# ypw0102/GDR

Measured on AMD Instinct MI355X. Metric: queries/sec on NQ-320k (768-d), higher is better.
Workload: dtype f32; 1 GPU; C2/ragged/prefilter: t5-base encoder 512 q/GPU + Q.D^T top-100, 320000x768 corpus; batch_per_gpu=512, global_batch=512, seq_len=40, corpus_rows=320000, dim=768, k=100, encoder_rows=ragged

## Files before the change

gdr_amd/csrc/encoder.hip:

```cpp
#include <stdlib.h>

#include "layers.h"

namespace gdr {

constexpr size_t ENC_SPLITK_BYTES = (size_t)112 << 20;
static_assert(STREAMK_BYTES <= ENC_SPLITK_BYTES, "stream-K scratch must fit the split-K region");

static int enc_streamk(char* splitk_region, StreamK* sk, hipStream_t stream) {
  sk->part = reinterpret_cast<float*>(splitk_region);
  sk->flag = reinterpret_cast<int32_t*>(splitk_region + STREAMK_PART_BYTES);
  sk->epoch = 0;
  if (hipMemsetAsync(sk->flag, 0, 512 * sizeof(int32_t), stream) != hipSuccess) {
    set_error("t5_encoder: memset of the stream-K flags failed");
    return GDR_EHIP;
  }
  return GDR_OK;
}

struct EncWs {
  size_t off_h, off_nx, off_qkv, off_ctx, off_ff, off_splitk, off_bf, total;
};

static EncWs enc_ws(const GdrT5Dims& dm, int64_t M, bool bf16 = false) {
// ... 97 lines not shown
        const __bf16* q16 = reinterpret_cast<const __bf16*>(qkv);
        at.q = reinterpret_cast<const float*>(q16), at.k = reinterpret_cast<const float*>(q16 + inner);
        at.v = reinterpret_cast<const float*>(q16 + 2 * inner), at.qkv_bf16 = 1;
      }
      at.out_bf16 = abf;
      if ((rc = launch_attention(at, stream))) return rc;
      if ((rc = lin16(abf, ly.wo, h, d, d, inner, 0, h, 0))) return rc;
      if ((rc = launch_rmsnorm_bf16(h, ly.ln_ff, abf, M, d, dm.eps, stream))) return rc;
      if ((rc = lin16(abf, ly.wi, ff, dm.d_ff, dm.d_ff, d, 1, nullptr, 1))) return rc;
      if ((rc = lin16(ff, ly.wo_ff, h, d, d, dm.d_ff, 0, h, 0))) return rc;
      continue;
    }
    if ((rc = launch_rmsnorm(h, ly.ln_attn, nx, M, d, dm.eps, nullptr, 1, stream))) return rc;
    if ((rc = linear(nx, d, ly.wqkv, qkv, 3 * inner, 3 * inner, d, GDR_EPI_NONE, nullptr))) return rc;
    if ((rc = launch_attention(at, stream))) return rc;
    if ((rc = linear(ctx, inner, ly.wo, h, d, d, inner, GDR_EPI_RESIDUAL, h))) return rc;
    if ((rc = launch_rmsnorm(h, ly.ln_ff, nx, M, d, dm.eps, nullptr, 1, stream))) return rc;
    if ((rc = linear(nx, d, ly.wi, ff, dm.d_ff, dm.d_ff, d, GDR_EPI_RELU, nullptr))) return rc;
    if ((rc = linear(ff, dm.d_ff, ly.wo_ff, h, d, d, dm.d_ff, GDR_EPI_RESIDUAL, h))) return rc;
  }
  return launch_rmsnorm(h, w->final_ln, out_hidden, M, d, dm.eps, out_pooled, L, stream);
}
}

extern "C" int gdr_t5_encoder_forward(const GdrT5EncoderWeights* w, const int64_t* ids, const int64_t* mask, int B,
                                      int L, float* out_hidden, float* out_pooled, void* workspace,
                                      size_t workspace_bytes, void* stream_) {
  return gdr::t5_encoder_impl(w, ids, mask, B, L, out_hidden, out_pooled, workspace, workspace_bytes, false,
                              static_cast<hipStream_t>(stream_));
}

namespace gdr {
struct RagWs {
  size_t seq_len, seq_off, row_src, rows_total, ctx_cls, h_cls, nx_cls, ff_cls, total;
};
static RagWs rag_ws(const GdrT5Dims& dm, int B, int L, size_t base) {
  RagWs r{};
  const size_t inner = (size_t)dm.num_heads * dm.d_kv;
  size_t o = base;
  r.seq_len = o, o += align_up((size_t)B * 4, 256);
  r.seq_off = o, o += align_up((size_t)(B + 1) * 4, 256);
  r.row_src = o, o += align_up((size_t)B * L * 4, 256);
  r.rows_total = o, o += 256;
  r.ctx_cls = o, o += align_up((size_t)B * inner * 4, 256);
  r.h_cls = o, o += align_up((size_t)B * dm.d_model * 4, 256);
  r.nx_cls = o, o += align_up((size_t)B * dm.d_model * 4, 256);
  r.ff_cls = o, o += align_up((size_t)B * dm.d_ff * 4, 256);
  r.total = o;
  return r;
}
static bool ragged_packs(const GdrT5Dims& dm, int B, int L) {
  const int64_t tiles = (((int64_t)B * L + 127) / 128) * ((dm.d_model + 127) / 128);
  return dm.d_kv == 64 && tiles >= 192 && dm.d_model % 32 == 0 && dm.d_ff % 32 == 0 && (dm.num_heads * dm.d_kv) % 32 == 0;
}
static bool ragged_packs_small(const GdrT5Dims& dm, int B, int L) {
  return dm.d_kv == 64 && (int64_t)B * L >= 256 && dm.d_model % 32 == 0 && dm.d_ff % 32 == 0 && (dm.num_heads * dm.d_kv) % 32 == 0;
}
}

extern "C" size_t gdr_t5_encoder_ragged_workspace_bytes(const GdrT5Dims* dims, int B, int L) {
  if (!dims || B <= 0 || L <= 0) return 0;
  return gdr::rag_ws(*dims, B, L, gdr::enc_ws(*dims, (int64_t)B * L, true).total).total;
}

namespace gdr {
static int ragged_impl(const GdrT5EncoderWeights* w, const int64_t* ids, const int64_t* mask, int B, int L, float* out_hidden,
                       float* out_pooled, int64_t live_rows_hint, void* workspace, size_t workspace_bytes, bool bf16,
                       hipStream_t stream) {
  if (B == 0) return GDR_OK;
  GDR_CHECK_ARG(w && ids && mask && workspace && (out_hidden || out_pooled), "t5_encoder_ragged: null pointer");
  const GdrT5Dims& dm = w->dims;
  GDR_CHECK_ARG(B > 0 && L > 0 && L <= 128, "t5_encoder_ragged: B=%d L=%d (L must be in [1,128])", B, L);
  GDR_CHECK_ARG(dm.d_model % 4 == 0 && dm.d_kv % 4 == 0 && dm.d_ff % 4 == 0, "t5_encoder_ragged: dims must be multiples of 4");
  GDR_CHECK_ARG(w->embed && w->rel_bias && w->final_ln && w->layers, "t5_encoder_ragged: null weight pointer");
  const int64_t M = (int64_t)B * L;
  const EncWs ws = enc_ws(dm, M, true);
  const RagWs rw = rag_ws(dm, B, L, ws.total);
  if (workspace_bytes < rw.total) {
    set_error("t5_encoder_ragged: workspace %zu < required %zu", workspace_bytes, rw.total);
    return GDR_ENOSPC;
// ... 65 lines not shown
          return rc;
        if ((rc = launch_gather_rows(h, seq_off, B, d, h_cls, stream))) return rc;
        if ((rc = lin16(ctx_cls16, ly.wo, h_cls, d, B, nullptr, d, inner, 0, h_cls, 0))) return rc;
        if ((rc = launch_rmsnorm_bf16(h_cls, ly.ln_ff, nx_cls16, B, d, dm.eps, stream))) return rc;
        if ((rc = lin16(nx_cls16, ly.wi, static_cast<float*>(ff_cls16), dm.d_ff, B, nullptr, dm.d_ff, d, 1, nullptr, 1))) return rc;
        if ((rc = lin16(ff_cls16, ly.wo_ff, h_cls, d, B, nullptr, d, dm.d_ff, 0, h_cls, 0))) return rc;
        return launch_rmsnorm(h_cls, w->final_ln, out_pooled, B, d, dm.eps, nullptr, 1, stream);
      }
      if ((rc = lin16(abf, ly.wo, h, d, M, rows_dev, d, inner, 0, h, 0))) return rc;
      if ((rc = launch_rmsnorm_bf16_dev(h, ly.ln_ff, abf, rows_dev, M, d, dm.eps, stream))) return rc;
      if ((rc = lin16(abf, ly.wi, ff, dm.d_ff, M, rows_dev, dm.d_ff, d, 1, nullptr, 1))) return rc;
      if ((rc = lin16(ff, ly.wo_ff, h, d, M, rows_dev, d, dm.d_ff, 0, h, 0))) return rc;
    }
    if ((rc = launch_rmsnorm_dev(h, w->final_ln, nx, rows_dev, M, d, dm.eps, stream))) return rc;
    if (out_pooled && (rc = launch_gather_rows(nx, seq_off, B, d, out_pooled, stream))) return rc;
    if (out_hidden) {
      if (hipMemsetAsync(out_hidden, 0, (size_t)M * d * sizeof(float), stream) != hipSuccess) {
        set_error("t5_encoder_ragged: memset failed");
        return GDR_EHIP;
      }
      if ((rc = launch_scatter_rows(nx, row_src, rows_dev, M, d, out_hidden, stream))) return rc;
    }
    return GDR_OK;
  }
  float* h = reinterpret_cast<float*>(base + ws.off_h);
  float* nx = reinterpret_cast<float*>(base + ws.off_nx);
  float* qkv = reinterpret_cast<float*>(base + ws.off_qkv);
  float* ctx = reinterpret_cast<float*>(base + ws.off_ctx);
  float* ff = reinterpret_cast<float*>(base + ws.off_ff);
  float* ctx_cls = reinterpret_cast<float*>(base + rw.ctx_cls);
  float* h_cls = reinterpret_cast<float*>(base + rw.h_cls);
  float* nx_cls = reinterpret_cast<float*>(base + rw.nx_cls);
  float* ff_cls = reinterpret_cast<float*>(base + rw.ff_cls);
  StreamK sk{};
  if ((rc = enc_streamk(base + ws.off_splitk, &sk, stream))) return rc;
  float* skw = reinterpret_cast<float*>(base + ws.off_splitk);
  auto linear = [&](const float* A, int64_t lda, const float* W, float* C, int64_t ldc, int N, int K, int epi,
                    const float* residual) -> int {
    if (small)
      return launch_linear_f32_ws(A, lda, W, K, C, ldc, M, N, K, epi, nullptr, residual, ldc, skw, ENC_SPLITK_BYTES, stream, &sk,
                                  rows_dev, live_rows_hint);
    return launch_linear_f32_dev(A, lda, W, K, C, ldc, M, rows_dev, N, K, epi, nullptr, residual, ldc, live_rows_hint, stream,
                                 &sk);
  };
  if ((rc = launch_embed_packed(w->embed, ids, row_src, rows_dev, M, d, dm.vocab_size, h, stream))) return rc;

  AttnArgs at{};
  at.q = qkv, at.k = qkv + inner, at.v = qkv + 2 * inner, at.out = ctx;
  at.ldq = at.ldk = at.ldv = 3 * inner, at.ldo = inner;
  at.q_bstride = at.k_bstride = at.o_bstride = L;
  at.B = B, at.H = H, at.dk = dk, at.Lq = L, at.Lk = L;
  at.q_pos0 = 0, at.scale = 1.0f;
  at.rel_bias = w->rel_bias, at.bidirectional = 1, at.num_buckets = dm.rel_buckets;
  at.lut = make_bucket_lut(dm.rel_buckets / 2, dm.rel_max_distance);
  at.key_mask = mask, at.mask_bstride = L, at.causal = 0, at.causal_neg_inf = 0;
  at.kv_rows = nullptr, at.kv_group = 1;
  at.seq_off = seq_off, at.seq_len = seq_len;

  const bool pooled_only = out_hidden == nullptr && big;
  for (int i = 0; i < dm.num_layers; ++i) {
    const GdrT5EncLayer& ly = w->layers[i];
    GDR_CHECK_ARG(ly.ln_attn && ly.wqkv && ly.wo && ly.ln_ff && ly.wi && ly.wo_ff, "t5_encoder_ragged: layer %d null weight", i);
    if ((rc = launch_rmsnorm_dev(h, ly.ln_attn, nx, rows_dev, M, d, dm.eps, stream))) return rc;
    if ((rc = linear(nx, d, ly.wqkv, qkv, 3 * inner, 3 * inner, d, GDR_EPI_NONE, nullptr))) return rc;
    if ((rc = launch_attention(at, stream))) return rc;
    if (pooled_only && i == dm.num_layers - 1) {
      if ((rc = launch_gather_rows(ctx, seq_off, B, inner, ctx_cls, stream))) return rc;
      if ((rc = launch_gather_rows(h, seq_off, B, d, h_cls, stream))) return rc;
      if ((rc = launch_linear_f32(ctx_cls, inner, ly.wo, inner, h_cls, d, B, d, inner, GDR_EPI_RESIDUAL, nullptr, h_cls, d, stream)))
        return rc;
      if ((rc = launch_rmsnorm(h_cls, ly.ln_ff, nx_cls, B, d, dm.eps, nullptr, 1, stream))) return rc;
      if ((rc = launch_linear_f32(nx_cls, d, ly.wi, d, ff_cls, dm.d_ff, B, dm.d_ff, d, GDR_EPI_RELU, nullptr, nullptr, 0, stream)))
        return rc;
      if ((rc = launch_linear_f32(ff_cls, dm.d_ff, ly.wo_ff, dm.d_ff, h_cls, d, B, d, dm.d_ff, GDR_EPI_RESIDUAL, nullptr, h_cls, d,
                                  stream)))
        return rc;
      return launch_rmsnorm(h_cls, w->final_ln, out_pooled, B, d, dm.eps, nullptr, 1, stream);
    }
    if ((rc = linear(ctx, inner, ly.wo, h, d, d, inner, GDR_EPI_RESIDUAL, h))) return rc;
    if ((rc = launch_rmsnorm_dev(h, ly.ln_ff, nx, rows_dev, M, d, dm.eps, stream))) return rc;
    if ((rc = linear(nx, d, ly.wi, ff, dm.d_ff, dm.d_ff, d, GDR_EPI_RELU, nullptr))) return rc;
    if ((rc = linear(ff, dm.d_ff, ly.wo_ff, h, d, d, dm.d_ff, GDR_EPI_RESIDUAL, h))) return rc;
  }
  if ((rc = launch_rmsnorm_dev(h, w->final_ln, nx, rows_dev, M, d, dm.eps, stream))) return rc;
  if (out_pooled && (rc = launch_gather_rows(nx, seq_off, B, d, out_pooled, stream))) return rc;
  if (out_hidden) {
    if (hipMemsetAsync(out_hidden, 0, (size_t)M * d * sizeof(float), stream) != hipSuccess) {
      set_error("t5_encoder_ragged: memset failed");
      return GDR_EHIP;
    }
    if ((rc = launch_scatter_rows(nx, row_src, rows_dev, M, d, out_hidden, stream))) return rc;
  }
  return GDR_OK;
}
}

namespace gdr {
static size_t split_ws_a_bytes(const GdrT5Dims& dm, int64_t M) {
  const int inner = dm.num_heads * dm.d_kv;
  int ld = split_row_elems(dm.d_model);
  if (split_row_elems(inner) > ld) ld = split_row_elems(inner);
  return align_up((size_t)M * ld * 2, 256);
}
static size_t split_ws_bytes(const GdrT5Dims& dm, int64_t M) {
  return split_ws_a_bytes(dm, M) + align_up((size_t)M * split_row_elems(dm.d_ff) * 2, 256);
}

static int ragged_split_impl(const GdrT5EncoderWeights* w, const int64_t* ids, const int64_t* mask, int B, int L, float* out_hidden,
                             float* out_pooled, int64_t live_rows_hint, int terms, void* workspace, size_t workspace_bytes,
                             hipStream_t stream) {
  if (B == 0) return GDR_OK;
// ... 161 lines not shown
```

gdr_amd/csrc/layers.h:

```cpp
#pragma once
#include "common.h"

namespace gdr {

struct BucketLut {
  uint8_t v[128];
};
BucketLut make_bucket_lut(int nb, int max_distance);

struct AttnArgs {
  const float* q;
  const float* k;
  const float* v;
  float* out;
  void* out_bf16;
  int64_t ldq, ldk, ldv, ldo;
  int64_t q_bstride, k_bstride, o_bstride;
  int B, H, dk, Lq, Lk;
  int q_pos0;
  float scale;
  const float* rel_bias;
  int bidirectional, num_buckets;
  BucketLut lut;
  const int64_t* key_mask;
  int64_t mask_bstride;
  int causal;
  int causal_neg_inf;
  const int32_t* kv_rows;
  int kv_group;
  int q_same_pos;
  const int32_t* seq_off;
  const int32_t* seq_len;
  int qkv_bf16;
  const int64_t* b_count_dev;
  const float* q_part;
  int q_S, q_tiles_n;
  const int32_t* live;
};
int launch_attention(const AttnArgs& a, hipStream_t stream);
int launch_attention_long(const AttnArgs& a, hipStream_t stream);

int launch_embed(const float* table, const int64_t* ids, int64_t rows, int d, int vocab, float* out,
                 hipStream_t stream);
int launch_pack_plan(const int64_t* mask, int B, int L, int32_t* seq_len, int32_t* seq_off, int32_t* row_src,
                     int64_t* rows_total, hipStream_t stream);
int launch_embed_packed(const float* table, const int64_t* ids, const int32_t* row_src, const int64_t* rows_dev,
                        int64_t max_rows, int d, int vocab, float* out, hipStream_t stream);
int launch_gather_rows(const float* src, const int32_t* idx, int n, int d, float* dst, hipStream_t stream);
int launch_scatter_rows(const float* src, const int32_t* row_src, const int64_t* rows_dev, int64_t max_rows, int d,
                        float* dst, hipStream_t stream);
int launch_rmsnorm(const float* x, const float* w, float* y, int64_t rows, int d, float eps, float* pooled,
                   int pool_every, hipStream_t stream, void* y16 = nullptr);
int launch_zero_dead_rows(float* x, const int32_t* seq_len, int B, int L, int d, hipStream_t stream);
int launch_rmsnorm_dev(const float* x, const float* w, float* y, const int64_t* rows_dev, int64_t max_rows, int d, float eps,
                       hipStream_t stream, void* y16 = nullptr);
int launch_rmsnorm_planes(const float* x, const float* w, float* y, void* planes, int64_t ld, const int64_t* rows_dev, int64_t max_rows,
                          int d, float eps, hipStream_t stream, int f16x2 = 0);
int launch_rmsnorm_bf16(const float* x, const float* w, void* y_bf16, int64_t rows, int d, float eps, hipStream_t stream);
int launch_rmsnorm_bf16_dev(const float* x, const float* w, void* y_bf16, const int64_t* rows_dev, int64_t max_rows, int d,
                            float eps, hipStream_t stream);
int launch_layernorm(const float* x, const float* w, const float* b, float* y, int64_t rows, int d, float eps,
                     const float* addv, hipStream_t stream, void* y16 = nullptr, int f16x2_ld = 0);
int launch_layernorm_dev(const float* x, const float* w, const float* b, float* y, const int64_t* rows_dev, int64_t max_rows,
                         int d, float eps, const float* addv, hipStream_t stream, void* y16 = nullptr, int f16x2_ld = 0);
int launch_layernorm2(const float* x, const float* w1, const float* b1, const float* w2, const float* b2, const float* addv, float* y,
                      const int64_t* rows_dev, int64_t max_rows, int d, float eps, hipStream_t stream, void* y16 = nullptr);
// ... 3 lines not shown
```

gdr_amd/csrc/layers.hip:

```cpp
#include <math.h>

#include <stdlib.h>

#include "layers.h"

namespace gdr {

BucketLut make_bucket_lut(int nb, int max_distance) {
  BucketLut l;
  const int max_exact = nb / 2;
  for (int n = 0; n < 128; ++n) {
    int b;
    if (n < max_exact) {
      b = n;
    } else {
      const float v = logf((float)n / (float)max_exact) / (float)log((double)max_distance / max_exact) *
                      (float)(nb - max_exact);
      b = max_exact + (int)v;
      if (b > nb - 1) b = nb - 1;
    }
    l.v[n] = (uint8_t)b;
  }
  return l;
}
// ... 611 lines not shown
        }
      }
      sum = wave_sum(sum);
      sc[0] = sum;
    }
    __builtin_amdgcn_wave_barrier();
    if (active) {
      const float inv = 1.0f / sc[0];
      float* orow = a.out + ((int64_t)b * a.o_bstride + i) * a.ldo + h * dk;
      for (int d = lane; d < dk; d += 64) {
        float o = 0.f;
        int j = 0;
        for (; j + 4 <= Lk; j += 4) {
          const float4 pp = *reinterpret_cast<const float4*>(ps + j);
          o = fmaf(pp.x * inv, Vs[(j + 0) * dks + d], o);
          o = fmaf(pp.y * inv, Vs[(j + 1) * dks + d], o);
          o = fmaf(pp.z * inv, Vs[(j + 2) * dks + d], o);
          o = fmaf(pp.w * inv, Vs[(j + 3) * dks + d], o);
        }
        for (; j < Lk; ++j) o = fmaf(ps[j] * inv, Vs[j * dks + d], o);
        if (a.out_bf16)
          static_cast<__bf16*>(a.out_bf16)[((int64_t)b * a.o_bstride + i) * a.ldo + h * dk + d] = (__bf16)o;
        else
          orow[d] = o;
      }
    }
    __builtin_amdgcn_wave_barrier();
  }
}


typedef float f32x4_t __attribute__((ext_vector_type(4)));

template <int NT>
__global__ __launch_bounds__(64 * NT) void attention_mfma16_kernel(const AttnArgs a) {
  extern __shared__ __attribute__((aligned(16))) float smem[];
  constexpr int DK = 64, DS = DK + 4, LP = 16 * NT, NTHR = 64 * NT;
  const int Lr = a.Lk;
  float* Ks = smem;
  float* Vs = Ks + Lr * DS;
  float* RelB = Vs + Lr * DS;
  float* Mk = RelB + 2 * LP;
  const int b = blockIdx.x / a.H, h = blockIdx.x % a.H;
  const int L = a.seq_len ? a.seq_len[b] : a.Lk, tid = threadIdx.x;
  const int64_t qrow0 = a.seq_off ? a.seq_off[b] : (int64_t)b * a.q_bstride;
  const int64_t krow0 = a.seq_off ? a.seq_off[b] : (int64_t)b * a.k_bstride;
  const int64_t orow0 = a.seq_off ? a.seq_off[b] : (int64_t)b * a.o_bstride;
  float4 qv[DK / 16];
  {
    const int wq = tid >> 6, lq = tid & 63;
    const int64_t qr = qrow0 + min(16 * wq + (lq & 15), L - 1);
    if (16 * wq < L) {
      if (a.qkv_bf16) {
        const __bf16* q16 = reinterpret_cast<const __bf16*>(a.q) + qr * a.ldq + h * DK + 4 * (lq >> 4);
#pragma unroll
        for (int jj = 0; jj < DK / 16; ++jj) {
          const uint2 u = *reinterpret_cast<const uint2*>(q16 + 16 * jj);
          qv[jj] = make_float4(__uint_as_float(u.x << 16) * a.scale, __uint_as_float(u.x & 0xffff0000u) * a.scale,
                               __uint_as_float(u.y << 16) * a.scale, __uint_as_float(u.y & 0xffff0000u) * a.scale);
        }
      } else {
        const float* q32 = a.q + qr * a.ldq + h * DK + 4 * (lq >> 4);
#pragma unroll
        for (int jj = 0; jj < DK / 16; ++jj) qv[jj] = *reinterpret_cast<const float4*>(q32 + 16 * jj);
      }
    }
  }
  int rb_bucket = -1;
  int rb_lutoff[2];
  unsigned char rb_lut[2] = {0, 0};
  int rb_base[2] = {0, 0};
  constexpr int RBI = (2 * LP + NTHR - 1) / NTHR;
  static_assert(RBI == 1, "one bias cell per thread");
  if (a.rel_bias && tid < 2 * LP) {
    int n = tid - (LP - 1), bucket = 0;
    if (a.bidirectional) {
      if (n < 0) {
        bucket = a.num_buckets >> 1;
        n = -n;
      }
    } else if (n < 0) {
      n = 0;
    }
    rb_base[0] = bucket;
    rb_lutoff[0] = n < 127 ? n : 127;
// ... 34 lines not shown
    }
    __builtin_amdgcn_sched_barrier(0);
    asm volatile("" ::: "memory");
    float rb_val = 0.f;
    if (rb_bucket >= 0) rb_val = a.rel_bias[(rb_base[0] + rb_lut[0]) * a.H + h];
    __builtin_amdgcn_sched_barrier(0);
    asm volatile("" ::: "memory");
#pragma unroll
    for (int it = 0; it < KI; ++it) {
      asm volatile("" : "+v"(kst[it].x), "+v"(kst[it].y), "+v"(kst[it].z), "+v"(kst[it].w));
      asm volatile("" : "+v"(vst[it].x), "+v"(vst[it].y), "+v"(vst[it].z), "+v"(vst[it].w));
    }
    asm volatile("" : "+v"(mk_raw));
#pragma unroll
    for (int it = 0; it < KI; ++it) {
      const int e = tid + it * NTHR;
      if (e < L * (DK / 4)) {
        const int r = e >> 4, c = e & 15;
        *reinterpret_cast<float4*>(Ks + r * DS + 4 * c) = kst[it];
        *reinterpret_cast<float4*>(Vs + r * DS + 4 * c) = vst[it];
      }
    }
    if (tid < 2 * LP) RelB[tid] = rb_val;
  }
  if (a.qkv_bf16 && tid < 2 * LP) RelB[tid] = rb_bucket >= 0 ? a.rel_bias[(rb_base[0] + rb_lut[0]) * a.H + h] : 0.f;
  if (tid < LP) Mk[tid] = tid < L ? ((mk_mine && mk_raw == 0) ? (a.causal_neg_inf ? -INFINITY : -1e9f) : 0.f) : -INFINITY;
  __syncthreads();
  if (!a.qkv_bf16) {
#pragma unroll
    for (int jj = 0; jj < DK / 16; ++jj) qv[jj].x *= a.scale, qv[jj].y *= a.scale, qv[jj].z *= a.scale, qv[jj].w *= a.scale;
  }

  const int w = tid >> 6, lane = tid & 63, c16 = lane & 15, q4 = lane >> 4;
  if (16 * w >= L) return;
  const int nt_live = (L + 15) >> 4;
  f32x4_t st[NT];
#pragma unroll
  for (int t = 0; t < NT; ++t) st[t] = (f32x4_t){0.f, 0.f, 0.f, 0.f};
#pragma unroll
  for (int jj = 0; jj < DK / 16; ++jj) {
#pragma unroll
    for (int t = 0; t < NT; ++t) {
      if (t >= nt_live) continue;
      const float4 kv = *reinterpret_cast<const float4*>(Ks + min(16 * t + c16, L - 1) * DS + 4 * q4 + 16 * jj);
      st[t] = __builtin_amdgcn_mfma_f32_16x16x4f32(kv.x, qv[jj].x, st[t], 0, 0, 0);
      st[t] = __builtin_amdgcn_mfma_f32_16x16x4f32(kv.y, qv[jj].y, st[t], 0, 0, 0);
      st[t] = __builtin_amdgcn_mfma_f32_16x16x4f32(kv.z, qv[jj].z, st[t], 0, 0, 0);
      st[t] = __builtin_amdgcn_mfma_f32_16x16x4f32(kv.w, qv[jj].w, st[t], 0, 0, 0);
    }
  }
  const int i = 16 * w + c16;
  const float masked = a.causal_neg_inf ? -INFINITY : -1e9f;
  float mx = -INFINITY;
#pragma unroll
  for (int t = 0; t < NT; ++t) {
    if (t >= nt_live) continue;
#pragma unroll
    for (int r = 0; r < 4; ++r) {
      const int j = 16 * t + 4 * q4 + r;
      float add = RelB[i - j + (LP - 1)] + Mk[j];
      if (a.causal && j > i && Mk[j] == 0.f) add += masked;
      const float s = st[t][r] + add;
      st[t][r] = s;
      mx = fmaxf(mx, s);
    }
  }
  mx = fmaxf(mx, __shfl_xor(mx, 16));
  mx = fmaxf(mx, __shfl_xor(mx, 32));
  float sum = 0.f;
#pragma unroll
  for (int t = 0; t < NT; ++t) {
    if (t >= nt_live) continue;
#pragma unroll
    for (int r = 0; r < 4; ++r) {
      const float p = __expf(st[t][r] - mx);
      st[t][r] = p;
      sum += p;
    }
  }
  sum += __shfl_xor(sum, 16);
  sum += __shfl_xor(sum, 32);
  const float inv = 1.0f / sum;
#pragma unroll
  for (int dt = 0; dt < DK / 16; ++dt) {
    f32x4_t o = (f32x4_t){0.f, 0.f, 0.f, 0.f};
#pragma unroll
    for (int t = 0; t < NT; ++t) {
      if (t >= nt_live) continue;
#pragma unroll
      for (int r = 0; r < 4; ++r) {
        const int j = 16 * t + 4 * q4 + r;
        const float vv = Vs[min(j, L - 1) * DS + 16 * dt + c16];
        o = __builtin_amdgcn_mfma_f32_16x16x4f32(vv, st[t][r], o, 0, 0, 0);
      }
    }
    if (i < L) {
      const int64_t off = (orow0 + i) * a.ldo + h * DK + 16 * dt + 4 * q4;
      const float4 ov = make_float4(o[0] * inv, o[1] * inv, o[2] * inv, o[3] * inv);
      if (a.out_bf16)
        *reinterpret_cast<uint2*>(static_cast<__bf16*>(a.out_bf16) + off) = pack_bf16x4(ov.x, ov.y, ov.z, ov.w);
      else
        *reinterpret_cast<float4*>(a.out + off) = ov;
    }
  }
}

typedef __bf16 bf16x8_t __attribute__((ext_vector_type(8)));

__device__ __forceinline__ uint32_t bf16_trunc_bits(float x) { return __float_as_uint(x) & 0xffff0000u; }

template <int NT>
__global__ __launch_bounds__(64 * NT) void attention_mfma_bf16_kernel(const AttnArgs a) {
  extern __shared__ __attribute__((aligned(16))) unsigned char smem_b[];
  constexpr int DK = 64, KS = 144, VS = 272, LP = 16 * NT, NTHR = 64 * NT, NB = (NT + 1) / 2, VKEYS = 32 * NB;
  const int Lr = a.Lk;
  unsigned char* Ks = smem_b;
  unsigned char* Vt = Ks + (size_t)((Lr * KS + 15) & ~15);
  float* RelB = reinterpret_cast<float*>(Vt + DK * VS);
  float* Mk = RelB + 2 * LP;
  const int b = blockIdx.x / a.H, h = blockIdx.x % a.H;
  const int L = a.seq_len ? a.seq_len[b] : a.Lk, tid = threadIdx.x;
  const int64_t qrow0 = a.seq_off ? a.seq_off[b] : (int64_t)b * a.q_bstride;
  const int64_t krow0 = a.seq_off ? a.seq_off[b] : (int64_t)b * a.k_bstride;
  const int64_t orow0 = a.seq_off ? a.seq_off[b] : (int64_t)b * a.o_bstride;
  const __bf16* q16 = reinterpret_cast<const __bf16*>(a.q);
  const __bf16* k16 = reinterpret_cast<const __bf16*>(a.k);
  const __bf16* v16 = reinterpret_cast<const __bf16*>(a.v);
  uint4 qv[2];
  {
    const int wq = tid >> 6, lq = tid & 63;
// ... 120 lines not shown
#pragma unroll
    for (int u = 0; u < NB; ++u) {
      if (2 * u >= nt_live) continue;
      const uint2 v0 = *reinterpret_cast<const uint2*>(vr + 64 * u);
      const uint2 v1 = *reinterpret_cast<const uint2*>(vr + 64 * u + 32);
      const bf16x8_t va = __builtin_bit_cast(bf16x8_t, make_uint4(v0.x, v0.y, v1.x, v1.y));
      o = __builtin_amdgcn_mfma_f32_16x16x32_bf16(va, __builtin_bit_cast(bf16x8_t, ph[u]), o, 0, 0, 0);
      o = __builtin_amdgcn_mfma_f32_16x16x32_bf16(va, __builtin_bit_cast(bf16x8_t, pm[u]), o, 0, 0, 0);
      o = __builtin_amdgcn_mfma_f32_16x16x32_bf16(va, __builtin_bit_cast(bf16x8_t, pl[u]), o, 0, 0, 0);
    }
    if (i < L) {
      const int64_t off = (orow0 + i) * a.ldo + h * DK + 16 * dt + 4 * q4;
      const float4 ov = make_float4(o[0] * inv, o[1] * inv, o[2] * inv, o[3] * inv);
      if (a.out_bf16)
        *reinterpret_cast<uint2*>(static_cast<__bf16*>(a.out_bf16) + off) = pack_bf16x4(ov.x, ov.y, ov.z, ov.w);
      else
        *reinterpret_cast<float4*>(a.out + off) = ov;
    }
  }
}

template <int NT>
static int launch_attention_mfma_bf16(const AttnArgs& a, hipStream_t stream) {
  const size_t lds = (size_t)((a.Lk * 144 + 15) & ~15) + 64 * 272 + sizeof(float) * 3 * 16 * NT;
  if (int rc__ = ensure_dyn_lds(reinterpret_cast<const void*>(attention_mfma_bf16_kernel<NT>), 160 * 1024, "attention")) return rc__;
  hipLaunchKernelGGL(attention_mfma_bf16_kernel<NT>, dim3((unsigned)(a.B * a.H)), dim3(64 * NT), lds, stream, a);
  GDR_CHECK_LAUNCH("attention_mfma_bf16_kernel");
  return GDR_OK;
}

template <int NT>
static int launch_attention_mfma16(const AttnArgs& a, hipStream_t stream) {
  const size_t lds = sizeof(float) * ((size_t)2 * a.Lk * 68 + 3 * 16 * NT);
  if (int rc__ = ensure_dyn_lds(reinterpret_cast<const void*>(attention_mfma16_kernel<NT>), 160 * 1024, "attention")) return rc__;
  hipLaunchKernelGGL(attention_mfma16_kernel<NT>, dim3((unsigned)(a.B * a.H)), dim3(64 * NT), lds, stream, a);
  GDR_CHECK_LAUNCH("attention_mfma16_kernel");
  return GDR_OK;
}


template <int NT>
__global__ __launch_bounds__(512) void attention_cross_mfma16_kernel(const AttnArgs a) {
  extern __shared__ __attribute__((aligned(16))) float smem[];
  if (a.live && *a.live == 0) return;
  constexpr int DK = 64, DS = DK + 4, LP = 16 * NT;
  const int Lk = a.Lk, Lq = a.Lq;
  float* Ks = smem;
  float* Vs = Ks + Lk * DS;
  float* Add = Vs + Lk * DS;
  const int b = blockIdx.x / a.H, h = blockIdx.x % a.H;
  const int tid = threadIdx.x, nthr = blockDim.x;
  const int w = tid >> 6, lane = tid & 63, c16 = lane & 15, q4 = lane >> 4;
  const int64_t krow0 = (int64_t)(b / a.kv_group) * a.k_bstride;
  float4 qv[DK / 16];
  const bool has_rows = 16 * w < Lq;
  if (has_rows) {
    const int64_t qr = (int64_t)b * a.q_bstride + min(16 * w + c16, Lq - 1);
    const float* q32 = a.q + qr * a.ldq + h * DK + 4 * q4;
#pragma unroll
    for (int jj = 0; jj < DK / 16; ++jj) {
      float4 t = *reinterpret_cast<const float4*>(q32 + 16 * jj);
      t.x *= a.scale, t.y *= a.scale, t.z *= a.scale, t.w *= a.scale;
      qv[jj] = t;
    }
  }
  for (int j = tid; j < LP; j += nthr) {
// ... 415 lines not shown
          hipLaunchKernelGGL(attention_decode_heads4_kernel<4>, g4, dim3(256), 0, stream, a);
        else if (a.Lk <= 8)
          hipLaunchKernelGGL(attention_decode_heads4_kernel<8>, g4, dim3(256), 0, stream, a);
        else if (a.Lk <= 12)
          hipLaunchKernelGGL(attention_decode_heads4_kernel<12>, g4, dim3(256), 0, stream, a);
        else
          hipLaunchKernelGGL(attention_decode_heads4_kernel<16>, g4, dim3(256), 0, stream, a);
        GDR_CHECK_LAUNCH("attention_decode_heads4_kernel");
        return GDR_OK;
      }
#endif
      const dim3 grids((unsigned)((a.B * a.H + 3) / 4));
      if (a.dk <= 64)
        hipLaunchKernelGGL(attention_decode_short_kernel<16>, grids, dim3(256), 0, stream, a);
      else
        hipLaunchKernelGGL(attention_decode_short_kernel<32>, grids, dim3(256), 0, stream, a);
      GDR_CHECK_LAUNCH("attention_decode_short_kernel");
      return GDR_OK;
    }
    const dim3 grid((unsigned)((a.B * a.H + 3) / 4));
    if (a.dk <= 64)
      hipLaunchKernelGGL(attention_decode_rows_kernel<16>, grid, dim3(256), 0, stream, a);
    else
      hipLaunchKernelGGL(attention_decode_rows_kernel<32>, grid, dim3(256), 0, stream, a);
    GDR_CHECK_LAUNCH("attention_decode_rows_kernel");
    return GDR_OK;
  }
  const bool packed = a.seq_off != nullptr || a.qkv_bf16;
  GDR_CHECK_ARG(!a.seq_off || a.seq_len, "attention: seq_off without seq_len");
  GDR_CHECK_ARG(!packed || (a.Lq == a.Lk && a.q_pos0 == 0 && !a.kv_rows && a.kv_group == 1 && !a.q_same_pos &&
                            a.dk == 64 && a.ldo % 4 == 0),
                "attention: the packed (ragged) form and bf16 q/k/v serve full self-attention with d_kv = 64 only");
  GDR_CHECK_ARG(!a.qkv_bf16 || (a.ldq % 8 == 0 && a.ldk % 8 == 0 && a.ldv % 8 == 0), "attention: bf16 q/k/v need row strides %% 8 == 0");
  if (a.Lq == a.Lk && a.q_pos0 == 0 && !a.kv_rows && a.kv_group == 1 && !a.q_same_pos && a.dk == 64 && a.ldo % 4 == 0) {
    if (a.Lk > 128) return launch_attention_long(a, stream);
    if (a.qkv_bf16 && a.scale == 1.0f) {
      switch ((a.Lk + 15) / 16) {
        case 1: return launch_attention_mfma_bf16<1>(a, stream);
        case 2: return launch_attention_mfma_bf16<2>(a, stream);
        case 3: return launch_attention_mfma_bf16<3>(a, stream);
        case 4: return launch_attention_mfma_bf16<4>(a, stream);
        case 5: return launch_attention_mfma_bf16<5>(a, stream);
        case 6: return launch_attention_mfma_bf16<6>(a, stream);
        case 7: return launch_attention_mfma_bf16<7>(a, stream);
        default: return launch_attention_mfma_bf16<8>(a, stream);
      }
    }
    switch ((a.Lk + 15) / 16) {
      case 1: return launch_attention_mfma16<1>(a, stream);
      case 2: return launch_attention_mfma16<2>(a, stream);
      case 3: return launch_attention_mfma16<3>(a, stream);
      case 4: return launch_attention_mfma16<4>(a, stream);
      case 5: return launch_attention_mfma16<5>(a, stream);
      case 6: return launch_attention_mfma16<6>(a, stream);
      case 7: return launch_attention_mfma16<7>(a, stream);
      default: return launch_attention_mfma16<8>(a, stream);
    }
  }
  if (cross_mfma_wanted(a)) {
    switch ((a.Lk + 15) / 16) {
      case 1: return launch_attention_cross_mfma16<1>(a, stream);
      case 2: return launch_attention_cross_mfma16<2>(a, stream);
      case 3: return launch_attention_cross_mfma16<3>(a, stream);
      case 4: return launch_attention_cross_mfma16<4>(a, stream);
      case 5: return launch_attention_cross_mfma16<5>(a, stream);
      case 6: return launch_attention_cross_mfma16<6>(a, stream);
// ... 69 lines not shown
```

gdr_amd/csrc/sim_topk.hip:

```cpp
#include <stdlib.h>

#include "common.h"

namespace gdr {

constexpr int TILE = 128;
constexpr int SEL_THREADS = 256;

struct SimPlan {
  int64_t tiles_m;
  int stride;
  int64_t n_sample_tiles;
  int64_t n_slots;
  int64_t cap;
  size_t off_val, off_idx, off_cnt, off_thr, off_part, total;
};

static SimPlan make_plan(int B, int64_t N, int k, bool exhaustive) {
  SimPlan p{};
  p.tiles_m = (N + TILE - 1) / TILE;
  double target = sqrt((double)k * (double)N);
  if (target < k) target = k;
  int64_t ts = (int64_t)((target + TILE - 1) / TILE);
  if (ts < 1) ts = 1;
// ... 623 lines not shown
  const int ns_sel = (stream_mode && sliced_on && B <= 32) ? sliced_ns(p.cap, kpad) : 0;
  if (ns_thr) {
    sa.NS = ns_thr;
    ProfScope prof(PROF_SELECT, 0.0, stream);
    hipLaunchKernelGGL(sim_sliced_select_kernel<true>, dim3(B * ns_thr), dim3(SL_THREADS), 0, stream, sa);
    GDR_CHECK_LAUNCH("sim_sliced_select_kernel(threshold)");
  } else {
    hipLaunchKernelGGL(sim_threshold_kernel, dim3(B), dim3(sel_threads), 0, stream, ep.cand_val, p.cap, (int)p.n_slots,
                       k, thr, ep.cand_cnt, (const float*)nullptr);
    GDR_CHECK_LAUNCH("sim_threshold_kernel");
  }
  if (p.stride > 1) {
    ep.mode = 2;
    rc = stream_mode ? launch_sim_stream(D, N, Q, B, d, ep, bf16, stream) : launch_sim_gemm(D, N, Q, B, d, ep, bf16, stream);
    if (rc) return rc;
  }
  if (ns_sel) {
    sa.NS = ns_sel;
    ProfScope prof(PROF_SELECT, 0.0, stream);
    hipLaunchKernelGGL(sim_sliced_select_kernel<false>, dim3(B * ns_sel), dim3(SL_THREADS), 0, stream, sa);
    GDR_CHECK_LAUNCH("sim_sliced_select_kernel(select)");
    return GDR_OK;
  }
  hipLaunchKernelGGL(topk_select_kernel<false>, dim3(B), dim3(sel_threads), kpad * sizeof(unsigned long long), stream,
                     ep.cand_val, ep.cand_idx, ep.cand_cnt, p.cap, 1, B, k, kpad, idx_offset, (const float*)thr, out_val,
                     out_idx, status, 0, 1);
  GDR_CHECK_LAUNCH("topk_select_kernel");
  return GDR_OK;
}

namespace gdr {
__global__ __launch_bounds__(256) void sim_qprep_kernel(const float* __restrict__ Q, int d, float dnorm_max, __bf16* __restrict__ Q16,
                                                        float* __restrict__ eps2) {
  __shared__ float red[4];
  const int q = blockIdx.x;
  const float* row = Q + (int64_t)q * d;
  float ss = 0.f;
  for (int c = threadIdx.x * 4; c < d; c += 1024) {
    const float4 v = *reinterpret_cast<const float4*>(row + c);
    ss = fmaf(v.x, v.x, fmaf(v.y, v.y, fmaf(v.z, v.z, fmaf(v.w, v.w, ss))));
    union {
      __bf16 h[4];
      uint2 u;
    } o;
    o.h[0] = (__bf16)v.x, o.h[1] = (__bf16)v.y, o.h[2] = (__bf16)v.z, o.h[3] = (__bf16)v.w;
    *reinterpret_cast<uint2*>(Q16 + (int64_t)q * d + c) = o.u;
  }
#pragma unroll
  for (int off = 32; off > 0; off >>= 1) ss += __shfl_xor(ss, off);
  if ((threadIdx.x & 63) == 0) red[threadIdx.x >> 6] = ss;
  __syncthreads();
  if (threadIdx.x == 0) {
    const float nq = sqrtf(red[0] + red[1] + red[2] + red[3]) * 1.0001f;
    const float c = 0.0078125f + 1.52587890625e-5f + (float)d * 2.384185791015625e-7f;
    eps2[q] = 2.0f * nq * dnorm_max * c * 1.01f;
  }
}

__global__ __launch_bounds__(256) void row_norm2_max_kernel(const float* __restrict__ D, int64_t N, int d, unsigned* __restrict__ out) {
  const int lane = threadIdx.x & 63;
  float best = 0.f;
  for (int64_t r = (int64_t)blockIdx.x * 4 + (threadIdx.x >> 6); r < N; r += (int64_t)gridDim.x * 4) {
    const float* row = D + r * d;
    float ss = 0.f;
    for (int c = lane * 4; c < d; c += 256) {
      const float4 v = *reinterpret_cast<const float4*>(row + c);
      ss = fmaf(v.x, v.x, fmaf(v.y, v.y, fmaf(v.z, v.z, fmaf(v.w, v.w, ss))));
    }
#pragma unroll
    for (int off = 32; off > 0; off >>= 1) ss += __shfl_xor(ss, off);
    best = fmaxf(best, ss);
  }
  if (lane == 0) atomicMax(out, __float_as_uint(best));
}

template <int RC>
__global__ __launch_bounds__(1024) void prefilter_tail_kernel(const float* __restrict__ cand_val, const int32_t* __restrict__ cand_idx,
                                                              const int32_t* __restrict__ cand_cnt, int64_t cap, int k, int cap2,
                                                              int cap2p, const float* __restrict__ eps2, const float* __restrict__ Q,
                                                              const float* __restrict__ D, int d, int32_t idx_offset,
                                                              float* __restrict__ out_val, int32_t* __restrict__ out_idx,
                                                              int32_t* __restrict__ status) {
  __shared__ int hist[256];
  __shared__ int scan[256];
  __shared__ int res[2];
  __shared__ uint32_t red[32];
  __shared__ int n_sh;
  extern __shared__ __attribute__((aligned(16))) unsigned long long pkeys[];
// ... 54 lines not shown
    const int b = find_bin(hist, scan, need, &above, res);
    need -= above;
    prefix |= (uint32_t)b << shift;
    __syncthreads();
  }
  const float band = fkey_inv(nbits ? (prefix >> lsh) + lo : lo) - eps2[q];
  int32_t* ids = reinterpret_cast<int32_t*>(pkeys + cap2p / 2);
  if (tid == 0) n_sh = 0;
  __syncthreads();
  if (cached) {
#pragma unroll
    for (int u = 0; u < RC; ++u) {
      const int i = tid + u * 1024;
      if (rk[u] > kneg && fkey_inv(rk[u]) >= band) {
        const int32_t id = ix[i];
        if (id >= 0) {
          const int p = atomicAdd(&n_sh, 1);
          if (p < cap2) ids[p] = id;
        }
      }
    }
  } else {
    for (int i = tid; i < count; i += 1024) {
      const int32_t id = ix[i];
      if (id >= 0 && v[i] >= band) {
        const int p = atomicAdd(&n_sh, 1);
        if (p < cap2) ids[p] = id;
      }
    }
  }
  __syncthreads();
  const int n_all = n_sh, n2 = n_all < cap2 ? n_all : cap2;
  if (tid == 0 && status) status[q] = (c_all > (int)cap || n_all > cap2) ? 1 : 0;
  {
    constexpr int MAXP = 4;
    float4 qr[MAXP];
#pragma unroll
    for (int t = 0; t < MAXP; ++t) {
      const int col = lane * 4 + 256 * t;
      qr[t] = col < d ? *reinterpret_cast<const float4*>(Q + (int64_t)q * d + col) : make_float4(0.f, 0.f, 0.f, 0.f);
    }
    float* vals = reinterpret_cast<float*>(pkeys);
    for (int i0 = wave * 2; i0 < n2; i0 += 32) {
      const int i1 = i0 + 1 < n2 ? i0 + 1 : i0;
      const int64_t r0 = ids[i0], r1 = ids[i1];
      float4 a0[MAXP], a1[MAXP];
#pragma unroll
      for (int t = 0; t < MAXP; ++t) {
        const int col = lane * 4 + 256 * t;
        a0[t] = col < d ? *reinterpret_cast<const float4*>(D + r0 * d + col) : make_float4(0.f, 0.f, 0.f, 0.f);
        a1[t] = col < d ? *reinterpret_cast<const float4*>(D + r1 * d + col) : make_float4(0.f, 0.f, 0.f, 0.f);
      }
      float s0 = 0.f, s1 = 0.f;
#pragma unroll
      for (int t = 0; t < MAXP; ++t) {
        s0 = fmaf(qr[t].x, a0[t].x, s0), s0 = fmaf(qr[t].y, a0[t].y, s0), s0 = fmaf(qr[t].z, a0[t].z, s0), s0 = fmaf(qr[t].w, a0[t].w, s0);
        s1 = fmaf(qr[t].x, a1[t].x, s1), s1 = fmaf(qr[t].y, a1[t].y, s1), s1 = fmaf(qr[t].z, a1[t].z, s1), s1 = fmaf(qr[t].w, a1[t].w, s1);
      }
#pragma unroll
      for (int off = 32; off > 0; off >>= 1) s0 += __shfl_xor(s0, off), s1 += __shfl_xor(s1, off);
      if (lane == 0) {
        vals[i0] = s0;
        if (i1 != i0) vals[i1] = s1;
      }
    }
    __syncthreads();
    unsigned long long mykey[4];
#pragma unroll
    for (int u = 0; u < 4; ++u) {
      const int i = tid + u * 1024;
      mykey[u] = 0ull;
      if (i < n2) mykey[u] = ((unsigned long long)fkey(vals[i]) << 32) | (unsigned long long)(0xFFFFFFFFu - (uint32_t)ids[i]);
    }
    __syncthreads();
#pragma unroll
    for (int u = 0; u < 4; ++u) {
      const int i = tid + u * 1024;
      if (i < cap2p) pkeys[i] = mykey[u];
    }
    __syncthreads();
  }
  for (int size = 2; size <= cap2p; size <<= 1) {
    for (int stride = size >> 1; stride > 0; stride >>= 1) {
      for (int t = tid; t < (cap2p >> 1); t += 1024) {
        const int lo_i = (t / stride) * (stride << 1) + (t % stride), hi_i = lo_i + stride;
        const bool desc = ((lo_i & size) == 0);
        const unsigned long long a = pkeys[lo_i], b = pkeys[hi_i];
        if ((a < b) == desc) pkeys[lo_i] = b, pkeys[hi_i] = a;
      }
      __syncthreads();
    }
  }
  for (int i = tid; i < k; i += 1024) {
    const unsigned long long key = pkeys[i];
    float val = -INFINITY;
    int32_t id = -1;
    if (i < n2 && key != 0ull) {
      val = fkey_inv((uint32_t)(key >> 32));
      id = (int32_t)(0xFFFFFFFFu - (uint32_t)(key & 0xFFFFFFFFull)) + idx_offset;
    }
    out_val[(int64_t)q * k + i] = val;
    out_idx[(int64_t)q * k + i] = id;
  }
}

static int prefilter_cap2(int k) {
  int c = 1024;
  while (c < 4 * k) c <<= 1;
  return c;
}
struct PrefilterPlan {
  SimPlan p;
  int cap2;
  size_t off_q16, off_eps, total;
};
static PrefilterPlan make_prefilter_plan(int B, int64_t N, int d, int k) {
  PrefilterPlan pp{};
  pp.p = make_plan(B, N, k, false);
  pp.cap2 = prefilter_cap2(k);
  size_t o = pp.p.total;
  pp.off_q16 = o, o += align_up((size_t)B * d * 2, 256);
  pp.off_eps = o, o += align_up((size_t)B * 4, 256);
  pp.total = o;
  return pp;
}
}

// ... 136 lines not shown
```

Baseline: 30290 queries/s.

## Compute last-layer attention for CLS query only and tighten prefilter rescoring

In the pooled-only ragged encoder path, the last layer now projects K/V for all rows but Q only for the gathered CLS rows, and runs a CLS-only attention variant that uses a single wave per head. The prefilter also gets a tighter bf16 error bound that uses the measured quantization error, which should shrink the candidate band. The exact rescoring loop now keeps four rows in flight per wave, and the bitonic sort covers only the next power of two above the live candidate count instead of the full capacity. These changes touch three separate kernels and make the encoder path and the error bound more complex.

Measured after the change: 30580 queries/s, median of 6. About the same (+1.0%).

```diff
diff --git a/gdr_amd/csrc/encoder.hip b/gdr_amd/csrc/encoder.hip
--- a/gdr_amd/csrc/encoder.hip
+++ b/gdr_amd/csrc/encoder.hip
@@ -153,7 +153,7 @@
 
 namespace gdr {
 struct RagWs {
-  size_t seq_len, seq_off, row_src, rows_total, ctx_cls, h_cls, nx_cls, ff_cls, total;
+  size_t seq_len, seq_off, row_src, rows_total, ctx_cls, h_cls, nx_cls, ff_cls, q_cls, total;
 };
 static RagWs rag_ws(const GdrT5Dims& dm, int B, int L, size_t base) {
   RagWs r{};
@@ -167,6 +167,7 @@
   r.h_cls = o, o += align_up((size_t)B * dm.d_model * 4, 256);
   r.nx_cls = o, o += align_up((size_t)B * dm.d_model * 4, 256);
   r.ff_cls = o, o += align_up((size_t)B * dm.d_ff * 4, 256);
+  r.q_cls = o, o += align_up((size_t)B * inner * 4, 256);
   r.total = o;
   return r;
 }
@@ -298,6 +299,7 @@
   float* h_cls = reinterpret_cast<float*>(base + rw.h_cls);
   float* nx_cls = reinterpret_cast<float*>(base + rw.nx_cls);
   float* ff_cls = reinterpret_cast<float*>(base + rw.ff_cls);
+  float* q_cls = reinterpret_cast<float*>(base + rw.q_cls);
   StreamK sk{};
   if ((rc = enc_streamk(base + ws.off_splitk, &sk, stream))) return rc;
   float* skw = reinterpret_cast<float*>(base + ws.off_splitk);
@@ -328,10 +330,14 @@
     const GdrT5EncLayer& ly = w->layers[i];
     GDR_CHECK_ARG(ly.ln_attn && ly.wqkv && ly.wo && ly.ln_ff && ly.wi && ly.wo_ff, "t5_encoder_ragged: layer %d null weight", i);
     if ((rc = launch_rmsnorm_dev(h, ly.ln_attn, nx, rows_dev, M, d, dm.eps, stream))) return rc;
-    if ((rc = linear(nx, d, ly.wqkv, qkv, 3 * inner, 3 * inner, d, GDR_EPI_NONE, nullptr))) return rc;
-    if ((rc = launch_attention(at, stream))) return rc;
     if (pooled_only && i == dm.num_layers - 1) {
-      if ((rc = launch_gather_rows(ctx, seq_off, B, inner, ctx_cls, stream))) return rc;
+      if ((rc = linear(nx, d, ly.wqkv + (int64_t)inner * d, qkv + inner, 3 * inner, 2 * inner, d, GDR_EPI_NONE, nullptr))) return rc;
+      if ((rc = launch_gather_rows(nx, seq_off, B, d, nx_cls, stream))) return rc;
+      if ((rc = launch_linear_f32(nx_cls, d, ly.wqkv, d, q_cls, inner, B, inner, d, GDR_EPI_NONE, nullptr, nullptr, 0, stream)))
+        return rc;
+      AttnArgs ac = at;
+      ac.q = q_cls, ac.ldq = inner, ac.out = ctx_cls, ac.ldo = inner, ac.cls_query = 1;
+      if ((rc = launch_attention(ac, stream))) return rc;
       if ((rc = launch_gather_rows(h, seq_off, B, d, h_cls, stream))) return rc;
       if ((rc = launch_linear_f32(ctx_cls, inner, ly.wo, inner, h_cls, d, B, d, inner, GDR_EPI_RESIDUAL, nullptr, h_cls, d, stream)))
         return rc;
@@ -343,6 +349,8 @@
         return rc;
       return launch_rmsnorm(h_cls, w->final_ln, out_pooled, B, d, dm.eps, nullptr, 1, stream);
     }
+    if ((rc = linear(nx, d, ly.wqkv, qkv, 3 * inner, 3 * inner, d, GDR_EPI_NONE, nullptr))) return rc;
+    if ((rc = launch_attention(at, stream))) return rc;
     if ((rc = linear(ctx, inner, ly.wo, h, d, d, inner, GDR_EPI_RESIDUAL, h))) return rc;
     if ((rc = launch_rmsnorm_dev(h, ly.ln_ff, nx, rows_dev, M, d, dm.eps, stream))) return rc;
     if ((rc = linear(nx, d, ly.wi, ff, dm.d_ff, dm.d_ff, d, GDR_EPI_RELU, nullptr))) return rc;
diff --git a/gdr_amd/csrc/layers.h b/gdr_amd/csrc/layers.h
--- a/gdr_amd/csrc/layers.h
+++ b/gdr_amd/csrc/layers.h
@@ -32,6 +32,7 @@
   const int32_t* seq_off;
   const int32_t* seq_len;
   int qkv_bf16;
+  int cls_query;
   const int64_t* b_count_dev;
   const float* q_part;
   int q_S, q_tiles_n;
diff --git a/gdr_amd/csrc/layers.hip b/gdr_amd/csrc/layers.hip
--- a/gdr_amd/csrc/layers.hip
+++ b/gdr_amd/csrc/layers.hip
@@ -667,7 +667,7 @@
 
 typedef float f32x4_t __attribute__((ext_vector_type(4)));
 
-template <int NT>
+template <int NT, bool CLS = false>
 __global__ __launch_bounds__(64 * NT) void attention_mfma16_kernel(const AttnArgs a) {
   extern __shared__ __attribute__((aligned(16))) float smem[];
   constexpr int DK = 64, DS = DK + 4, LP = 16 * NT, NTHR = 64 * NT;
@@ -684,8 +684,8 @@
   float4 qv[DK / 16];
   {
     const int wq = tid >> 6, lq = tid & 63;
-    const int64_t qr = qrow0 + min(16 * wq + (lq & 15), L - 1);
-    if (16 * wq < L) {
+    const int64_t qr = CLS ? (int64_t)b : qrow0 + min(16 * wq + (lq & 15), L - 1);
+    if (16 * wq < L && (!CLS || wq == 0)) {
       if (a.qkv_bf16) {
         const __bf16* q16 = reinterpret_cast<const __bf16*>(a.q) + qr * a.ldq + h * DK + 4 * (lq >> 4);
 #pragma unroll
@@ -786,7 +786,7 @@
   }
 
   const int w = tid >> 6, lane = tid & 63, c16 = lane & 15, q4 = lane >> 4;
-  if (16 * w >= L) return;
+  if (16 * w >= L || (CLS && w > 0)) return;
   const int nt_live = (L + 15) >> 4;
   f32x4_t st[NT];
 #pragma unroll
@@ -848,8 +848,8 @@
         o = __builtin_amdgcn_mfma_f32_16x16x4f32(vv, st[t][r], o, 0, 0, 0);
       }
     }
-    if (i < L) {
-      const int64_t off = (orow0 + i) * a.ldo + h * DK + 16 * dt + 4 * q4;
+    if (CLS ? c16 == 0 : i < L) {
+      const int64_t off = (CLS ? (int64_t)b : orow0 + i) * a.ldo + h * DK + 16 * dt + 4 * q4;
       const float4 ov = make_float4(o[0] * inv, o[1] * inv, o[2] * inv, o[3] * inv);
       if (a.out_bf16)
         *reinterpret_cast<uint2*>(static_cast<__bf16*>(a.out_bf16) + off) = pack_bf16x4(ov.x, ov.y, ov.z, ov.w);
@@ -1036,6 +1036,12 @@
 template <int NT>
 static int launch_attention_mfma16(const AttnArgs& a, hipStream_t stream) {
   const size_t lds = sizeof(float) * ((size_t)2 * a.Lk * 68 + 3 * 16 * NT);
+  if (a.cls_query) {
+    if (int rc__ = ensure_dyn_lds(reinterpret_cast<const void*>(attention_mfma16_kernel<NT, true>), 160 * 1024, "attention")) return rc__;
+    hipLaunchKernelGGL((attention_mfma16_kernel<NT, true>), dim3((unsigned)(a.B * a.H)), dim3(64 * NT), lds, stream, a);
+    GDR_CHECK_LAUNCH("attention_mfma16_kernel(cls)");
+    return GDR_OK;
+  }
   if (int rc__ = ensure_dyn_lds(reinterpret_cast<const void*>(attention_mfma16_kernel<NT>), 160 * 1024, "attention")) return rc__;
   hipLaunchKernelGGL(attention_mfma16_kernel<NT>, dim3((unsigned)(a.B * a.H)), dim3(64 * NT), lds, stream, a);
   GDR_CHECK_LAUNCH("attention_mfma16_kernel");
@@ -1517,6 +1523,8 @@
                             a.dk == 64 && a.ldo % 4 == 0),
                 "attention: the packed (ragged) form and bf16 q/k/v serve full self-attention with d_kv = 64 only");
   GDR_CHECK_ARG(!a.qkv_bf16 || (a.ldq % 8 == 0 && a.ldk % 8 == 0 && a.ldv % 8 == 0), "attention: bf16 q/k/v need row strides %% 8 == 0");
+  GDR_CHECK_ARG(!a.cls_query || (packed && !a.qkv_bf16 && a.Lk <= 128),
+                "attention: the CLS-query form serves the packed fp32 self-attention (d_kv = 64, L <= 128) only");
   if (a.Lq == a.Lk && a.q_pos0 == 0 && !a.kv_rows && a.kv_group == 1 && !a.q_same_pos && a.dk == 64 && a.ldo % 4 == 0) {
     if (a.Lk > 128) return launch_attention_long(a, stream);
     if (a.qkv_bf16 && a.scale == 1.0f) {
diff --git a/gdr_amd/csrc/sim_topk.hip b/gdr_amd/csrc/sim_topk.hip
--- a/gdr_amd/csrc/sim_topk.hip
+++ b/gdr_amd/csrc/sim_topk.hip
@@ -679,10 +679,10 @@
 namespace gdr {
 __global__ __launch_bounds__(256) void sim_qprep_kernel(const float* __restrict__ Q, int d, float dnorm_max, __bf16* __restrict__ Q16,
                                                         float* __restrict__ eps2) {
-  __shared__ float red[4];
+  __shared__ float red[8];
   const int q = blockIdx.x;
   const float* row = Q + (int64_t)q * d;
-  float ss = 0.f;
+  float ss = 0.f, se = 0.f;
   for (int c = threadIdx.x * 4; c < d; c += 1024) {
     const float4 v = *reinterpret_cast<const float4*>(row + c);
     ss = fmaf(v.x, v.x, fmaf(v.y, v.y, fmaf(v.z, v.z, fmaf(v.w, v.w, ss))));
@@ -692,15 +692,19 @@
     } o;
     o.h[0] = (__bf16)v.x, o.h[1] = (__bf16)v.y, o.h[2] = (__bf16)v.z, o.h[3] = (__bf16)v.w;
     *reinterpret_cast<uint2*>(Q16 + (int64_t)q * d + c) = o.u;
-  }
-#pragma unroll
-  for (int off = 32; off > 0; off >>= 1) ss += __shfl_xor(ss, off);
-  if ((threadIdx.x & 63) == 0) red[threadIdx.x >> 6] = ss;
+    const float ex = (float)o.h[0] - v.x, ey = (float)o.h[1] - v.y, ez = (float)o.h[2] - v.z, ew = (float)o.h[3] - v.w;
+    se = fmaf(ex, ex, fmaf(ey, ey, fmaf(ez, ez, fmaf(ew, ew, se))));
+  }
+#pragma unroll
+  for (int off = 32; off > 0; off >>= 1) ss += __shfl_xor(ss, off), se += __shfl_xor(se, off);
+  if ((threadIdx.x & 63) == 0) red[threadIdx.x >> 6] = ss, red[4 + (threadIdx.x >> 6)] = se;
   __syncthreads();
   if (threadIdx.x == 0) {
     const float nq = sqrtf(red[0] + red[1] + red[2] + red[3]) * 1.0001f;
     const float c = 0.0078125f + 1.52587890625e-5f + (float)d * 2.384185791015625e-7f;
-    eps2[q] = 2.0f * nq * dnorm_max * c * 1.01f;
+    const float ne = sqrtf(red[4] + red[5] + red[6] + red[7]) * 1.0001f;
+    const float eps = fminf(nq * c, ne * 1.00390625f + nq * (0.00390625f + (float)d * 2.384185791015625e-7f)) * dnorm_max;
+    eps2[q] = 2.0f * eps * 1.01f;
   }
 }
 
@@ -821,6 +825,8 @@
   __syncthreads();
   const int n_all = n_sh, n2 = n_all < cap2 ? n_all : cap2;
   if (tid == 0 && status) status[q] = (c_all > (int)cap || n_all > cap2) ? 1 : 0;
+  int sp = 1;
+  while (sp < n2) sp <<= 1;
   {
     constexpr int MAXP = 4;
     float4 qr[MAXP];
@@ -830,27 +836,37 @@
       qr[t] = col < d ? *reinterpret_cast<const float4*>(Q + (int64_t)q * d + col) : make_float4(0.f, 0.f, 0.f, 0.f);
     }
     float* vals = reinterpret_cast<float*>(pkeys);
-    for (int i0 = wave * 2; i0 < n2; i0 += 32) {
-      const int i1 = i0 + 1 < n2 ? i0 + 1 : i0;
-      const int64_t r0 = ids[i0], r1 = ids[i1];
-      float4 a0[MAXP], a1[MAXP];
-#pragma unroll
-      for (int t = 0; t < MAXP; ++t) {
-        const int col = lane * 4 + 256 * t;
-        a0[t] = col < d ? *reinterpret_cast<const float4*>(D + r0 * d + col) : make_float4(0.f, 0.f, 0.f, 0.f);
-        a1[t] = col < d ? *reinterpret_cast<const float4*>(D + r1 * d + col) : make_float4(0.f, 0.f, 0.f, 0.f);
-      }
-      float s0 = 0.f, s1 = 0.f;
-#pragma unroll
-      for (int t = 0; t < MAXP; ++t) {
-        s0 = fmaf(qr[t].x, a0[t].x, s0), s0 = fmaf(qr[t].y, a0[t].y, s0), s0 = fmaf(qr[t].z, a0[t].z, s0), s0 = fmaf(qr[t].w, a0[t].w, s0);
-        s1 = fmaf(qr[t].x, a1[t].x, s1), s1 = fmaf(qr[t].y, a1[t].y, s1), s1 = fmaf(qr[t].z, a1[t].z, s1), s1 = fmaf(qr[t].w, a1[t].w, s1);
-      }
-#pragma unroll
-      for (int off = 32; off > 0; off >>= 1) s0 += __shfl_xor(s0, off), s1 += __shfl_xor(s1, off);
+    constexpr int RIF = 4;
+    for (int i0 = wave * RIF; i0 < n2; i0 += 16 * RIF) {
+      int64_t r[RIF];
+#pragma unroll
+      for (int j = 0; j < RIF; ++j) r[j] = ids[i0 + j < n2 ? i0 + j : i0];
+      float4 a[RIF][MAXP];
+#pragma unroll
+      for (int j = 0; j < RIF; ++j)
+#pragma unroll
+        for (int t = 0; t < MAXP; ++t) {
+          const int col = lane * 4 + 256 * t;
+          a[j][t] = col < d ? *reinterpret_cast<const float4*>(D + r[j] * d + col) : make_float4(0.f, 0.f, 0.f, 0.f);
+        }
+      __builtin_amdgcn_sched_barrier(0);
+      float sc[RIF];
+#pragma unroll
+      for (int j = 0; j < RIF; ++j) {
+        float s0 = 0.f;
+#pragma unroll
+        for (int t = 0; t < MAXP; ++t)
+          s0 = fmaf(qr[t].x, a[j][t].x, s0), s0 = fmaf(qr[t].y, a[j][t].y, s0), s0 = fmaf(qr[t].z, a[j][t].z, s0), s0 = fmaf(qr[t].w, a[j][t].w, s0);
+        sc[j] = s0;
+      }
+#pragma unroll
+      for (int off = 32; off > 0; off >>= 1)
+#pragma unroll
+        for (int j = 0; j < RIF; ++j) sc[j] += __shfl_xor(sc[j], off);
       if (lane == 0) {
-        vals[i0] = s0;
-        if (i1 != i0) vals[i1] = s1;
+#pragma unroll
+        for (int j = 0; j < RIF; ++j)
+          if (i0 + j < n2) vals[i0 + j] = sc[j];
       }
     }
     __syncthreads();
@@ -865,13 +881,13 @@
 #pragma unroll
     for (int u = 0; u < 4; ++u) {
       const int i = tid + u * 1024;
-      if (i < cap2p) pkeys[i] = mykey[u];
-    }
-    __syncthreads();
-  }
-  for (int size = 2; size <= cap2p; size <<= 1) {
+      if (i < sp) pkeys[i] = mykey[u];
+    }
+    __syncthreads();
+  }
+  for (int size = 2; size <= sp; size <<= 1) {
     for (int stride = size >> 1; stride > 0; stride >>= 1) {
-      for (int t = tid; t < (cap2p >> 1); t += 1024) {
+      for (int t = tid; t < (sp >> 1); t += 1024) {
         const int lo_i = (t / stride) * (stride << 1) + (t % stride), hi_i = lo_i + stride;
         const bool desc = ((lo_i & size) == 0);
         const unsigned long long a = pkeys[lo_i], b = pkeys[hi_i];
@@ -881,7 +897,7 @@
     }
   }
   for (int i = tid; i < k; i += 1024) {
-    const unsigned long long key = pkeys[i];
+    const unsigned long long key = i < n2 ? pkeys[i] : 0ull;
     float val = -INFINITY;
     int32_t id = -1;
     if (i < n2 && key != 0ull) {
```
